# wangrui2025/GDKVM

Measured on AMD Instinct MI355X. Metric: frames/sec (GDKVM forward + argmax mask), EchoNet 112x112x32 clips, higher is better.
Workload: dtype bf16; 1 GPU; BASELINE.json configs[1]: EchoNet-Dynamic 112x112x32 bf16 inference, batch=16 per GPU; clips_per_gpu=16, frames_per_clip=32, image=112x112, heads=1, key_dim=64, rule=delta_sequential, world_size=1, ranks_seen=1

## Files before the change

### gdkvm_amd/csrc/stem_conv_pool.hip

```cpp
#include <atomic>
#include "gdkvm_common.hpp"

namespace {

constexpr int SP_TPY = 4, SP_TPX = 28;
constexpr int SP_CR = 2 * SP_TPY + 1;
constexpr int SP_CC = 64;
constexpr int SP_BR = SP_CR + 3, SP_BC = SP_CC + 3;
constexpr int SP_SLOTS = SP_BR * SP_BC * 2;
constexpr int SP_PIECES = (SP_SLOTS + 63) / 64;
constexpr int SP_BAND_BYTES = SP_PIECES * 1024;
constexpr int SP_CPIX = 144;
constexpr int SP_CONV_BYTES = SP_CR * SP_CC * SP_CPIX;

__device__ const uint4 g_stem_zero16 = {0, 0, 0, 0};

struct StemArgs {
    const bf16_t* xs; const bf16_t* w; const float* bias; bf16_t* y;
    int N, Hs, Ws, Hp, Wp, tiles_x, tiles_y;
    const bf16_t* xf; int Cf;
};

template <bool NCHW, bool POOL = true>
__global__ __launch_bounds__(512, 1) void stem_conv_pool_kernel(StemArgs a)
{
    extern __shared__ __attribute__((aligned(16))) unsigned char smem[];
    unsigned char* band2 = smem;
    unsigned char* ctile = smem + 2 * SP_BAND_BYTES;
    const int tid = threadIdx.x, lane = tid & 63, li = lane & 15, g = lane >> 4;
    const int w = __builtin_amdgcn_readfirstlane(tid >> 6), wn = w & 1, wm = w >> 1;
    const int ntiles = a.N * a.tiles_y * a.tiles_x;

    bf16x8 wf[2][8];
#pragma unroll
    for (int nt = 0; nt < 2; ++nt)
#pragma unroll
        for (int ks = 0; ks < 8; ++ks) {
            const int co = 32 * wn + 8 * (li >> 2) + 4 * nt + (li & 3);
            wf[nt][ks] = *reinterpret_cast<const bf16x8*>(a.w + (size_t)co * 256 + 32 * ks + 8 * g);
        }
    float bia[8];
    {
        const f32x4 b0 = *reinterpret_cast<const f32x4*>(a.bias + 32 * wn + 8 * g), b1 = *reinterpret_cast<const f32x4*>(a.bias + 32 * wn + 8 * g + 4);
        bia[0] = b0[0]; bia[1] = b0[1]; bia[2] = b0[2]; bia[3] = b0[3]; bia[4] = b1[0]; bia[5] = b1[1]; bia[6] = b1[2]; bia[7] = b1[3];
    }

    constexpr int PP = (SP_PIECES + 7) / 8;
    auto fetch = [&](int tile, int buf) __attribute__((always_inline)) {
        const int tx = tile % a.tiles_x, t2 = tile / a.tiles_x, ty = t2 % a.tiles_y, n = t2 / a.tiles_y;
        const int y0 = (POOL ? 2 * SP_TPY * ty - 1 : SP_CR * ty) - 2, x0 = (POOL ? 2 * SP_TPX * tx - 1 : (SP_CC - 7) * tx) - 2;
#pragma unroll
        for (int u = 0; u < PP; ++u) {
            const int j = w + 8 * u;
            if (j >= SP_PIECES) break;
            const int d = 64 * j + lane, pix = d >> 1, c = d & 1;
            const int by = pix / SP_BC, bx = pix - by * SP_BC, yy = y0 + by, xx = x0 + bx;
            const bool ok = pix < SP_BR * SP_BC && yy >= 0 && yy < a.Hs && xx >= 0 && xx < a.Ws;
            const bf16_t* src = ok ? a.xs + ((((size_t)n * a.Hs + yy) * a.Ws + xx) * 16 + c * 8) : reinterpret_cast<const bf16_t*>(&g_stem_zero16);
            __builtin_amdgcn_global_load_lds(src, reinterpret_cast<__attribute__((address_space(3))) void*>(
                reinterpret_cast<uintptr_t>(band2 + buf * SP_BAND_BYTES + 1024 * j)), 16, 0, 0);
        }
    };

    unsigned stage[PP][4];
    auto fetch_nchw = [&](int tile) __attribute__((always_inline)) {
        const int tx = tile % a.tiles_x, t2 = tile / a.tiles_x, ty = t2 % a.tiles_y, n = t2 / a.tiles_y;
        const int y0 = (POOL ? 2 * SP_TPY * ty - 1 : SP_CR * ty) - 2, x0 = (POOL ? 2 * SP_TPX * tx - 1 : (SP_CC - 7) * tx) - 2;
        const int H = 2 * a.Hs, W = 2 * a.Ws;
#pragma unroll
        for (int u = 0; u < PP; ++u) {
            const int j = w + 8 * u, d = 64 * j + lane, pix = d >> 1, half = d & 1;
            const int by = pix / SP_BC, bx = pix - by * SP_BC, yy = y0 + by, xx = x0 + bx;
            const bool ok = j < SP_PIECES && pix < SP_BR * SP_BC && yy >= 0 && yy < a.Hs && xx >= 0 && xx < a.Ws;
#pragma unroll
            for (int e = 0; e < 4; ++e) {
                const int c = 2 * half + (e >> 1);
                const bool live = ok && c < a.Cf;
                const bf16_t* src = live ? a.xf + ((((size_t)n * a.Cf + c) * H + 2 * yy + (e & 1)) * W + 2 * xx) : reinterpret_cast<const bf16_t*>(&g_stem_zero16);
                stage[u][e] = *reinterpret_cast<const unsigned*>(src);
            }
        }
    };
    auto put_nchw = [&](int buf) __attribute__((always_inline)) {
#pragma unroll
        for (int u = 0; u < PP; ++u) {
            const int j = w + 8 * u;
            if (j < SP_PIECES)
                *reinterpret_cast<uint4*>(band2 + buf * SP_BAND_BYTES + 1024 * j + 16 * lane) = make_uint4(stage[u][0], stage[u][1], stage[u][2], stage[u][3]);
        }
    };

    const unsigned xoff = (unsigned)((16 * wm + li) * 32 + g * 16);
    int tile = blockIdx.x, cur = 0;
    if (tile < ntiles) {
        if constexpr (NCHW) { fetch_nchw(tile); put_nchw(0); }
        else fetch(tile, 0);
    }
    __syncthreads();
    for (; tile < ntiles; tile += gridDim.x, cur ^= 1) {
        const bool more = tile + (int)gridDim.x < ntiles;
        if (more) {
            if constexpr (NCHW) fetch_nchw(tile + gridDim.x);
            else fetch(tile + gridDim.x, cur ^ 1);
        }
        const unsigned char* band = band2 + cur * SP_BAND_BYTES;
        const int tx = tile % a.tiles_x, t2 = tile / a.tiles_x, ty = t2 % a.tiles_y, n = t2 / a.tiles_y;
        const int cy0 = POOL ? 2 * SP_TPY * ty - 1 : SP_CR * ty, cx0 = POOL ? 2 * SP_TPX * tx - 1 : (SP_CC - 7) * tx;
        const int cx = cx0 + 16 * wm + li;
        const bool col_ok = cx >= 0 && cx < a.Ws && (POOL || 16 * wm + li < SP_CC - 7);

#pragma unroll
        for (int grp = 0; grp < 3; ++grp) {
            f32x4 acc[3][2];
#pragma unroll
            for (int r = 0; r < 3; ++r) acc[r][0] = acc[r][1] = f32x4{0.f, 0.f, 0.f, 0.f};
            bf16x8 xf[6][2];
#pragma unroll
            for (int rho = 0; rho < 6; ++rho)
#pragma unroll
                for (int half = 0; half < 2; ++half)
                    xf[rho][half] = *reinterpret_cast<const bf16x8*>(band + xoff + ((3 * grp + rho) * SP_BC) * 32 + half * 64);
#pragma unroll
            for (int ks = 0; ks < 8; ++ks) {
                const int ky = ks >> 1, half = ks & 1;
#pragma unroll
                for (int r = 0; r < 3; ++r) {
                    acc[r][0] = __builtin_amdgcn_mfma_f32_16x16x32_bf16(wf[0][ks], xf[r + ky][half], acc[r][0], 0, 0, 0);
                    acc[r][1] = __builtin_amdgcn_mfma_f32_16x16x32_bf16(wf[1][ks], xf[r + ky][half], acc[r][1], 0, 0, 0);
                }
            }
            if constexpr (!POOL) {
#pragma unroll
                for (int r = 0; r < 3; ++r) {
                    const int cy = cy0 + 3 * grp + r;
                    if (col_ok && cy < a.Hs) {
                        unsigned ow[4];
#pragma unroll
                        for (int q = 0; q < 4; ++q)
                            ow[q] = (unsigned)f32_to_bf16(acc[r][q >> 1][2 * (q & 1)]) | ((unsigned)f32_to_bf16(acc[r][q >> 1][2 * (q & 1) + 1]) << 16);
                        *reinterpret_cast<uint4*>(a.y + (((size_t)n * a.Hs + cy) * a.Ws + cx) * 64 + 32 * wn + 8 * g) = make_uint4(ow[0], ow[1], ow[2], ow[3]);
                    }
                }
                continue;
            }
#pragma unroll
            for (int r = 0; r < 3; ++r) {
                const int cr = 3 * grp + r, cy = cy0 + cr;
                const float keep = (col_ok && cy >= 0 && cy < a.Hs) ? 1.f : 0.f;
                typedef float f32x2 __attribute__((ext_vector_type(2)));
                unsigned ow[4];
#pragma unroll
                for (int q = 0; q < 4; ++q) {
                    const f32x2 t = {acc[r][q >> 1][2 * (q & 1)], acc[r][q >> 1][2 * (q & 1) + 1]};
                    const f32x2 bb = {bia[2 * q], bia[2 * q + 1]};
                    f32x2 v = __builtin_elementwise_max(t + bb, f32x2{0.f, 0.f}) * f32x2{keep, keep};
                    ow[q] = (unsigned)f32_to_bf16(v[0]) | ((unsigned)f32_to_bf16(v[1]) << 16);
                }
                *reinterpret_cast<uint4*>(ctile + (cr * SP_CC + 16 * wm + li) * SP_CPIX + (32 * wn + 8 * g) * 2) = make_uint4(ow[0], ow[1], ow[2], ow[3]);
            }
        }
        if constexpr (NCHW) { if (more) put_nchw(cur ^ 1); }
        __syncthreads();

        for (int it = tid; POOL && it < SP_TPY * SP_TPX * 8; it += 512) {
            const int cg = it & 7, pp = it >> 3, q = pp / SP_TPX, px = pp - q * SP_TPX;
            const int py_g = SP_TPY * ty + q, px_g = SP_TPX * tx + px;
            typedef unsigned short u16x2 __attribute__((ext_vector_type(2)));
            u16x2 m[4] = {u16x2{0, 0}, u16x2{0, 0}, u16x2{0, 0}, u16x2{0, 0}};
#pragma unroll
            for (int dy = 0; dy < 3; ++dy)
#pragma unroll
                for (int dx = 0; dx < 3; ++dx) {
                    const uint4 t = *reinterpret_cast<const uint4*>(ctile + ((2 * q + dy) * SP_CC + 2 * px + dx) * SP_CPIX + cg * 16);
                    m[0] = __builtin_elementwise_max(m[0], __builtin_bit_cast(u16x2, t.x));
                    m[1] = __builtin_elementwise_max(m[1], __builtin_bit_cast(u16x2, t.y));
                    m[2] = __builtin_elementwise_max(m[2], __builtin_bit_cast(u16x2, t.z));
                    m[3] = __builtin_elementwise_max(m[3], __builtin_bit_cast(u16x2, t.w));
                }
            if (py_g < a.Hp && px_g < a.Wp) {
                const uint4 o = {__builtin_bit_cast(unsigned, m[0]), __builtin_bit_cast(unsigned, m[1]), __builtin_bit_cast(unsigned, m[2]),
                                 __builtin_bit_cast(unsigned, m[3])};
                *reinterpret_cast<uint4*>(a.y + (((size_t)n * a.Hp + py_g) * a.Wp + px_g) * 64 + cg * 8) = o;
            }
        }
        if constexpr (POOL) __syncthreads();
    }
}

__global__ __launch_bounds__(256) void stem_pack_s2d_kernel(const float* w7, bf16_t* w4, int C, long long sk, long long sc, long long sr, long long ss)
{
    const int i = blockIdx.x * 256 + threadIdx.x;
    if (i >= 64 * 256) return;
    const int ch = i & 15, b = (i >> 4) & 3, a = (i >> 6) & 3, k = i >> 8;
    const int c = ch >> 2, p = (ch >> 1) & 1, q = ch & 1, u = 2 * (a - 2) + p + 3, v = 2 * (b - 2) + q + 3;
    float x = 0.f;
    if (c < C && u >= 0 && u <= 6 && v >= 0 && v <= 6) x = w7[k * sk + c * sc + u * sr + v * ss];
    w4[i] = f32_to_bf16(x);
}


constexpr int SW_TH = 4, SW_TW = 56;
constexpr int SW_BR = SW_TH + 3, SW_BC = SW_TW + 3;
constexpr int SW_BSLOTS = SW_BR * SW_BC * 2;
constexpr int SW_BPT = (SW_BSLOTS + 255) / 256;
constexpr int SW_BAND_BYTES = (SW_BSLOTS * 16 + 1023) / 1024 * 1024;
constexpr int SW_YPIX = 144;
constexpr int SW_YPIECES = (SW_TH * SW_TW * 9 + 63) / 64;
constexpr int SW_KSTEPS = SW_TH * SW_TW / 32;
static_assert(SW_TH * SW_TW % 32 == 0 && SW_TW % 4 == 0, "tiles are whole k-steps; four consecutive pixels never straddle a row");

struct StemWgradArgs { const bf16_t* xf; const bf16_t* dy; float* part; int N, Cf, Hs, Ws, tiles_x, tiles_y; };

__global__ __launch_bounds__(256, 3) void stem_wgrad_kernel(StemWgradArgs a)
{
    __shared__ __attribute__((aligned(16))) unsigned char s_band[SW_BAND_BYTES];
    __shared__ __attribute__((aligned(16))) unsigned char s_y[SW_YPIECES * 1024];
    const int tid = threadIdx.x, lane = tid & 63, li = lane & 15, g = lane >> 4;
    const int w = __builtin_amdgcn_readfirstlane(tid >> 6);
    const int q = li >> 2, p4 = (li & 3) * 4;
    const int ntiles = a.N * a.tiles_y * a.tiles_x;
    const int H = 2 * a.Hs, W = 2 * a.Ws;

    f32x4 acc[4][4];
#pragma unroll
    for (int kt = 0; kt < 4; ++kt)
#pragma unroll
        for (int b = 0; b < 4; ++b) acc[kt][b] = f32x4{0.f, 0.f, 0.f, 0.f};

    for (int tile = blockIdx.x; tile < ntiles; tile += gridDim.x) {
        const int tx = tile % a.tiles_x, t2 = tile / a.tiles_x, ty = t2 % a.tiles_y, n = t2 / a.tiles_y;
        const int cy0 = SW_TH * ty, cx0 = SW_TW * tx, y0 = cy0 - 2, x0 = cx0 - 2;
        unsigned stage[SW_BPT][4];
#pragma unroll
        for (int u = 0; u < SW_BPT; ++u) {
            const int d = 256 * u + tid, pix = d >> 1, half = d & 1;
            const int by = pix / SW_BC, bx = pix - by * SW_BC, yy = y0 + by, xx = x0 + bx;
            const bool ok = d < SW_BSLOTS && yy >= 0 && yy < a.Hs && xx >= 0 && xx < a.Ws;
#pragma unroll
            for (int e = 0; e < 4; ++e) {
                const int c = 2 * half + (e >> 1);
                const bool live = ok && c < a.Cf;
                const bf16_t* src = live ? a.xf + ((((size_t)n * a.Cf + c) * H + 2 * yy + (e & 1)) * W + 2 * xx) : reinterpret_cast<const bf16_t*>(&g_stem_zero16);
                stage[u][e] = *reinterpret_cast<const unsigned*>(src);
            }
        }
        __syncthreads();
        for (int j = w; j < SW_YPIECES; j += 4) {
            const int d = 64 * j + lane, pix = d / 9, c = d - 9 * pix;
            const int py = pix / SW_TW, px = pix - py * SW_TW, cy = cy0 + py, cx = cx0 + px;
            const bool ok = c < 8 && pix < SW_TH * SW_TW && cy < a.Hs && cx < a.Ws;
            const bf16_t* src = ok ? a.dy + ((((size_t)n * a.Hs + cy) * a.Ws + cx) * 64 + c * 8) : reinterpret_cast<const bf16_t*>(&g_stem_zero16);
            __builtin_amdgcn_global_load_lds(src, reinterpret_cast<__attribute__((address_space(3))) void*>(reinterpret_cast<uintptr_t>(s_y + 1024 * j)), 16, 0, 0);
        }
#pragma unroll
        for (int u = 0; u < SW_BPT; ++u) {
            const int d = 256 * u + tid;
            if (d < SW_BSLOTS) *reinterpret_cast<uint4*>(s_band + 16 * d) = make_uint4(stage[u][0], stage[u][1], stage[u][2], stage[u][3]);
        }
        __syncthreads();
#pragma unroll 1
        for (int s = 0; s < SW_KSTEPS; ++s) {
            unsigned ya[2], xa[2];
#pragma unroll
            for (int hf = 0; hf < 2; ++hf) {
                const int pp = 32 * s + 8 * g + 4 * hf + q, py = pp / SW_TW, px = pp - py * SW_TW;
                ya[hf] = (unsigned)(uintptr_t)(s_y + pp * SW_YPIX + p4 * 2);
                xa[hf] = (unsigned)(uintptr_t)(s_band + ((py + w) * SW_BC + px) * 32 + p4 * 2);
            }
            uint2 fa[4][2], fb[4][2];
#pragma unroll
            for (int kt = 0; kt < 4; ++kt)
#pragma unroll
                for (int hf = 0; hf < 2; ++hf) asm volatile("ds_read_b64_tr_b16 %0, %1" : "=&v"(fa[kt][hf]) : "v"(ya[hf] + 32 * kt) : "memory");
#pragma unroll
            for (int b = 0; b < 4; ++b)
#pragma unroll
                for (int hf = 0; hf < 2; ++hf) asm volatile("ds_read_b64_tr_b16 %0, %1" : "=&v"(fb[b][hf]) : "v"(xa[hf] + 32 * b) : "memory");
            asm volatile("s_waitcnt lgkmcnt(0)"
                         : "+v"(fa[0][0]), "+v"(fa[0][1]), "+v"(fa[1][0]), "+v"(fa[1][1]), "+v"(fa[2][0]), "+v"(fa[2][1]), "+v"(fa[3][0]), "+v"(fa[3][1]),
                           "+v"(fb[0][0]), "+v"(fb[0][1]), "+v"(fb[1][0]), "+v"(fb[1][1]), "+v"(fb[2][0]), "+v"(fb[2][1]), "+v"(fb[3][0]), "+v"(fb[3][1])
                         :: "memory");
#pragma unroll
            for (int b = 0; b < 4; ++b) {
                const bf16x8 bf = __builtin_bit_cast(bf16x8, make_uint4(fb[b][0].x, fb[b][0].y, fb[b][1].x, fb[b][1].y));
#pragma unroll
                for (int kt = 0; kt < 4; ++kt) {
                    const bf16x8 af = __builtin_bit_cast(bf16x8, make_uint4(fa[kt][0].x, fa[kt][0].y, fa[kt][1].x, fa[kt][1].y));
                    acc[kt][b] = __builtin_amdgcn_mfma_f32_16x16x32_bf16(af, bf, acc[kt][b], 0, 0, 0);
                }
            }
        }
    }
    float* out = a.part + (size_t)blockIdx.x * (64 * 256);
#pragma unroll
    for (int kt = 0; kt < 4; ++kt)
#pragma unroll
        for (int b = 0; b < 4; ++b)
#pragma unroll
            for (int r = 0; r < 4; ++r) out[((16 * kt + 4 * g + r) * 4 + w) * 64 + 16 * b + li] = acc[kt][b][r];
}

__global__ __launch_bounds__(512) void stem_wgrad_reduce_kernel(const float* part, float* dw, int gx, int C, long long sk, long long sc, long long sr, long long ss)
{
    __shared__ float s_sum[8][64];
    const int e = threadIdx.x & 63, sl = threadIdx.x >> 6;
    const int per = (gx + 7) / 8, b0 = sl * per, b1 = min(gx, b0 + per);
    const int i = blockIdx.x * 64 + e;
    float s8[8] = {0.f, 0.f, 0.f, 0.f, 0.f, 0.f, 0.f, 0.f};
    int b = b0;
    for (; b + 8 <= b1; b += 8)
#pragma unroll
        for (int j = 0; j < 8; ++j) s8[j] += part[(size_t)(b + j) * (64 * 256) + i];
    for (int j = 0; b < b1; ++b, ++j) s8[j] += part[(size_t)b * (64 * 256) + i];
    const float s = ((s8[0] + s8[1]) + (s8[2] + s8[3])) + ((s8[4] + s8[5]) + (s8[6] + s8[7]));
    s_sum[sl][e] = s;
    __syncthreads();
    if (sl == 0) {
        float t8 = 0.f;
#pragma unroll
        for (int j = 0; j < 8; ++j) t8 += s_sum[j][e];
        const int ch = i & 15, bb = (i >> 4) & 3, aa = (i >> 6) & 3, k = i >> 8;
        const int c = ch >> 2, p = (ch >> 1) & 1, qq = ch & 1, u = 2 * aa + p - 1, v = 2 * bb + qq - 1;
        if (c < C && u >= 0 && u <= 6 && v >= 0 && v <= 6) dw[k * sk + c * sc + u * sr + v * ss] = t8;
    }
}

}

static int stem_conv_pool_impl(const char* who, const void* xs, const void* xf, int Cf, const void* w, const float* bias, void* y,
                               int N, int Hs, int Ws, int io_dtype, void* stream, bool pool = true)
{
    if (io_dtype != GDKVM_BF16) return gdkvm_fail(GDKVM_ERR_DTYPE, "%s: only bf16 is implemented", who);
    if (N < 0 || Hs <= 0 || Ws <= 0) return gdkvm_fail(GDKVM_ERR_SHAPE, "%s: N=%d Hs=%d Ws=%d", who, N, Hs, Ws);
    if (N == 0) return GDKVM_OK;
    const void* x = xf ? xf : xs;
    if (!x || !w || (pool && !bias) || !y) return gdkvm_fail(GDKVM_ERR_ARG, "%s: null pointer", who);
    if (!gdkvm_aligned16(x) || !gdkvm_aligned16(w) || !gdkvm_aligned16(y) || (bias && !gdkvm_aligned16(bias)))
        return gdkvm_fail(GDKVM_ERR_ARG, "%s: pointers must be 16-byte aligned", who);
    if (int rc = gdkvm_check_device()) return rc;
    StemArgs a;
    a.xs = static_cast<const bf16_t*>(xs); a.w = static_cast<const bf16_t*>(w); a.bias = bias; a.y = static_cast<bf16_t*>(y);
    a.xf = static_cast<const bf16_t*>(xf); a.Cf = Cf;
    a.N = N; a.Hs = Hs; a.Ws = Ws; a.Hp = (Hs - 1) / 2 + 1; a.Wp = (Ws - 1) / 2 + 1;
    a.tiles_x = (a.Wp + SP_TPX - 1) / SP_TPX; a.tiles_y = (a.Hp + SP_TPY - 1) / SP_TPY;
    if (!pool) { a.tiles_x = (Ws + SP_CC - 8) / (SP_CC - 7); a.tiles_y = (Hs + SP_CR - 1) / SP_CR; }
    const long long ntiles = (long long)N * a.tiles_x * a.tiles_y;
    if (ntiles > 0x7fffffffLL) return gdkvm_fail(GDKVM_ERR_SHAPE, "%s: too many tiles", who);
    const size_t lds = 2 * (size_t)SP_BAND_BYTES + SP_CONV_BYTES;
    {
        static std::atomic<unsigned long long> done_mask{0};
        int dev = 0;
        if (hipGetDevice(&dev) != hipSuccess) return gdkvm_fail(GDKVM_ERR_LAUNCH, "%s: hipGetDevice", who);
        const unsigned long long bit = 1ull << (dev & 63);
        if (!(done_mask.load(std::memory_order_relaxed) & bit)) {
            hipError_t e = hipFuncSetAttribute(reinterpret_cast<const void*>(stem_conv_pool_kernel<false>), hipFuncAttributeMaxDynamicSharedMemorySize, (int)lds);
            if (e == hipSuccess) e = hipFuncSetAttribute(reinterpret_cast<const void*>(stem_conv_pool_kernel<true>), hipFuncAttributeMaxDynamicSharedMemorySize, (int)lds);
            if (e == hipSuccess) e = hipFuncSetAttribute(reinterpret_cast<const void*>(stem_conv_pool_kernel<true, false>), hipFuncAttributeMaxDynamicSharedMemorySize, (int)lds);
            if (e != hipSuccess) return gdkvm_fail(GDKVM_ERR_LAUNCH, "%s: %s", who, hipGetErrorString(e));
            done_mask.fetch_or(bit, std::memory_order_relaxed);
        }
    }
    constexpr int STEM_GRID = 256;
    const int grid = (int)(ntiles < STEM_GRID ? ntiles : STEM_GRID);
    if (!pool) hipLaunchKernelGGL((stem_conv_pool_kernel<true, false>), dim3(grid), dim3(512), lds, static_cast<hipStream_t>(stream), a);
    else if (xf) hipLaunchKernelGGL(stem_conv_pool_kernel<true>, dim3(grid), dim3(512), lds, static_cast<hipStream_t>(stream), a);
    else hipLaunchKernelGGL(stem_conv_pool_kernel<false>, dim3(grid), dim3(512), lds, static_cast<hipStream_t>(stream), a);
    GDKVM_LAUNCH_CHECK("stem_conv_pool_kernel");
    return GDKVM_OK;
}

extern "C" int gdkvm_stem_conv_pool(const void* xs, const void* w, const float* bias, void* y, int N, int Hs, int Ws,
                                    int io_dtype, void* stream)
{
    return stem_conv_pool_impl("stem_conv_pool", xs, nullptr, 0, w, bias, y, N, Hs, Ws, io_dtype, stream);
}

extern "C" int gdkvm_stem_conv_pool_nchw(const void* x, const void* w, const float* bias, void* y, int N, int C, int H, int W,
                                         int io_dtype, void* stream)
{
    if (C <= 0 || C > 4 || H <= 0 || W <= 0 || (H & 1) || (W & 1))
        return gdkvm_fail(GDKVM_ERR_SHAPE, "stem_conv_pool_nchw: C=%d H=%d W=%d (at most 4 channels, H and W even)", C, H, W);
    return stem_conv_pool_impl("stem_conv_pool_nchw", nullptr, x, C, w, bias, y, N, H / 2, W / 2, io_dtype, stream);
}

extern "C" int gdkvm_stem_conv_nchw(const void* x, const void* w4, void* y, int N, int C, int H, int W, int io_dtype, void* stream)
{
    if (C <= 0 || C > 4 || H <= 0 || W <= 0 || (H & 1) || (W & 1))
        return gdkvm_fail(GDKVM_ERR_SHAPE, "stem_conv_nchw: C=%d H=%d W=%d (at most 4 channels, H and W even)", C, H, W);
    return stem_conv_pool_impl("stem_conv_nchw", nullptr, x, C, w4, nullptr, y, N, H / 2, W / 2, io_dtype, stream, false);
}

extern "C" int gdkvm_stem_pack_s2d(const float* w7, void* w4, int C, long long sk, long long sc, long long sr, long long ss, void* stream)
{
    if (C <= 0 || C > 4) return gdkvm_fail(GDKVM_ERR_SHAPE, "stem_pack_s2d: C=%d (at most 4 input channels)", C);
    if (!w7 || !w4 || !gdkvm_aligned16(w4)) return gdkvm_fail(GDKVM_ERR_ARG, "stem_pack_s2d: null or unaligned pointer");
    if (int rc = gdkvm_check_device()) return rc;
    hipLaunchKernelGGL(stem_pack_s2d_kernel, dim3(64), dim3(256), 0, static_cast<hipStream_t>(stream), w7, static_cast<bf16_t*>(w4), C, sk, sc, sr, ss);
    GDKVM_LAUNCH_CHECK("stem_pack_s2d_kernel");
    return GDKVM_OK;
}


static int stem_wgrad_grid(int N, int Hs, int Ws, int* tiles_x, int* tiles_y)
{
    *tiles_x = (Ws + SW_TW - 1) / SW_TW; *tiles_y = (Hs + SW_TH - 1) / SW_TH;
    const long long ntiles = (long long)N * *tiles_x * *tiles_y;
    if (ntiles > 0x7fffffffLL) return -1;
    return (int)(ntiles < 768 ? ntiles : 768);
}

extern "C" size_t gdkvm_stem_wgrad_workspace_bytes(int N, int H, int W)
{
    int tx, ty;
    if (N <= 0 || H <= 0 || W <= 0) return 16;
    const int gx = stem_wgrad_grid(N, H / 2, W / 2, &tx, &ty);
    return gx <= 0 ? 16 : (size_t)gx * 64 * 256 * sizeof(float);
}

extern "C" int gdkvm_stem_wgrad_nchw(const void* x, const void* dy, float* dw, long long sk, long long sc, long long sr, long long ss,
                                     void* workspace, size_t workspace_bytes, int N, int C, int H, int W, int io_dtype, void* stream)
{
    if (io_dtype != GDKVM_BF16) return gdkvm_fail(GDKVM_ERR_DTYPE, "stem_wgrad_nchw: only bf16 operands are implemented");
    if (C <= 0 || C > 4 || H <= 0 || W <= 0 || (H & 1) || (W & 1) || N < 0)
        return gdkvm_fail(GDKVM_ERR_SHAPE, "stem_wgrad_nchw: N=%d C=%d H=%d W=%d (at most 4 channels, H and W even)", N, C, H, W);
    if (N == 0) return GDKVM_OK;
    if (!x || !dy || !dw || !workspace || !gdkvm_aligned16(x) || !gdkvm_aligned16(dy) || !gdkvm_aligned16(workspace))
        return gdkvm_fail(GDKVM_ERR_ARG, "stem_wgrad_nchw: null or unaligned pointer");
    StemWgradArgs a;
    a.xf = static_cast<const bf16_t*>(x); a.dy = static_cast<const bf16_t*>(dy); a.part = static_cast<float*>(workspace);
    a.N = N; a.Cf = C; a.Hs = H / 2; a.Ws = W / 2;
    const int gx = stem_wgrad_grid(N, a.Hs, a.Ws, &a.tiles_x, &a.tiles_y);
    if (gx <= 0) return gdkvm_fail(GDKVM_ERR_SHAPE, "stem_wgrad_nchw: too many tiles");
    const size_t need = (size_t)gx * 64 * 256 * sizeof(float);
    if (workspace_bytes < need) return gdkvm_fail(GDKVM_ERR_WORKSPACE, "stem_wgrad_nchw: workspace %zu < %zu bytes", workspace_bytes, need);
    if (int rc = gdkvm_check_device()) return rc;
    hipStream_t st = static_cast<hipStream_t>(stream);
    hipLaunchKernelGGL(stem_wgrad_kernel, dim3(gx), dim3(256), 0, st, a);
    GDKVM_LAUNCH_CHECK("stem_wgrad_kernel");
    hipLaunchKernelGGL(stem_wgrad_reduce_kernel, dim3(64 * 256 / 64), dim3(512), 0, st, static_cast<const float*>(workspace), dw, gx, C, sk, sc, sr, ss);
    GDKVM_LAUNCH_CHECK("stem_wgrad_reduce_kernel");
    return GDKVM_OK;
}
```

Baseline: 597,400 frames/s.

## Fuse stem maxpool into conv registers with row carry and DPP column max

The pooled stem kernel no longer writes the conv tile to LDS and reruns a separate pool pass. Each wave now folds conv rows straight into per-window row maxima held in registers, does the horizontal max across lanes with DPP shifts, and carries the last conv row into the next vertically adjacent tile. Tiles are handed to blocks in contiguous ranges ordered by tile row so the carry can be reused. The band is narrower (14 columns per wave), which cuts LDS use and removes the dynamic-LDS attribute setup, but lanes with odd index or index 14 and above go idle at store time, and the overlapping band columns mean some conv work is duplicated.

```diff
diff --git a/gdkvm_amd/csrc/stem_conv_pool.hip b/gdkvm_amd/csrc/stem_conv_pool.hip
--- a/gdkvm_amd/csrc/stem_conv_pool.hip
+++ b/gdkvm_amd/csrc/stem_conv_pool.hip
@@ -1,4 +1,4 @@
-#include <atomic>
+#include <type_traits>
 #include "gdkvm_common.hpp"
 
 namespace {
@@ -6,12 +6,18 @@
 constexpr int SP_TPY = 4, SP_TPX = 28;
 constexpr int SP_CR = 2 * SP_TPY + 1;
 constexpr int SP_CC = 64;
-constexpr int SP_BR = SP_CR + 3, SP_BC = SP_CC + 3;
+constexpr int SP_BR = SP_CR + 3;
+
+constexpr int SP_CS = 14;
+constexpr int SPP_BC = 3 * SP_CS + 16 + 3;
+constexpr int SPP_PIECES = (SP_BR * SPP_BC * 2 + 63) / 64;
+constexpr int SPP_BAND_BYTES = SPP_PIECES * 1024;
+static_assert(SP_TPX == 4 * (SP_CS / 2) && SP_CS % 2 == 0, "each wave pools SP_CS / 2 whole windows");
+
+constexpr int SP_BC = SP_CC + 3;
 constexpr int SP_SLOTS = SP_BR * SP_BC * 2;
 constexpr int SP_PIECES = (SP_SLOTS + 63) / 64;
 constexpr int SP_BAND_BYTES = SP_PIECES * 1024;
-constexpr int SP_CPIX = 144;
-constexpr int SP_CONV_BYTES = SP_CR * SP_CC * SP_CPIX;
 
 __device__ const uint4 g_stem_zero16 = {0, 0, 0, 0};
 
@@ -21,15 +27,16 @@
     const bf16_t* xf; int Cf;
 };
 
-template <bool NCHW, bool POOL = true>
+template <bool NCHW>
 __global__ __launch_bounds__(512, 1) void stem_conv_pool_kernel(StemArgs a)
 {
     extern __shared__ __attribute__((aligned(16))) unsigned char smem[];
     unsigned char* band2 = smem;
-    unsigned char* ctile = smem + 2 * SP_BAND_BYTES;
     const int tid = threadIdx.x, lane = tid & 63, li = lane & 15, g = lane >> 4;
     const int w = __builtin_amdgcn_readfirstlane(tid >> 6), wn = w & 1, wm = w >> 1;
     const int ntiles = a.N * a.tiles_y * a.tiles_x;
+    const int per = (ntiles + (int)gridDim.x - 1) / (int)gridDim.x;
+    const int t0 = (int)blockIdx.x * per, t1 = min(ntiles, t0 + per);
 
     bf16x8 wf[2][8];
 #pragma unroll
@@ -45,27 +52,180 @@
         bia[0] = b0[0]; bia[1] = b0[1]; bia[2] = b0[2]; bia[3] = b0[3]; bia[4] = b1[0]; bia[5] = b1[1]; bia[6] = b1[2]; bia[7] = b1[3];
     }
 
-    constexpr int PP = (SP_PIECES + 7) / 8;
-    auto fetch = [&](int tile, int buf) __attribute__((always_inline)) {
-        const int tx = tile % a.tiles_x, t2 = tile / a.tiles_x, ty = t2 % a.tiles_y, n = t2 / a.tiles_y;
-        const int y0 = (POOL ? 2 * SP_TPY * ty - 1 : SP_CR * ty) - 2, x0 = (POOL ? 2 * SP_TPX * tx - 1 : (SP_CC - 7) * tx) - 2;
+    auto where = [&](int t, int& n, int& ty, int& tx) __attribute__((always_inline)) {
+        ty = t % a.tiles_y; const int t2 = t / a.tiles_y; tx = t2 % a.tiles_x; n = t2 / a.tiles_x;
+    };
+    constexpr int PP = (SPP_PIECES + 7) / 8;
+    auto fetch = [&](int t, int buf) __attribute__((always_inline)) {
+        int n, ty, tx; where(t, n, ty, tx);
+        const int y0 = 2 * SP_TPY * ty - 3, x0 = 2 * SP_TPX * tx - 3;
 #pragma unroll
         for (int u = 0; u < PP; ++u) {
             const int j = w + 8 * u;
-            if (j >= SP_PIECES) break;
+            if (j >= SPP_PIECES) break;
             const int d = 64 * j + lane, pix = d >> 1, c = d & 1;
-            const int by = pix / SP_BC, bx = pix - by * SP_BC, yy = y0 + by, xx = x0 + bx;
-            const bool ok = pix < SP_BR * SP_BC && yy >= 0 && yy < a.Hs && xx >= 0 && xx < a.Ws;
+            const int by = pix / SPP_BC, bx = pix - by * SPP_BC, yy = y0 + by, xx = x0 + bx;
+            const bool ok = pix < SP_BR * SPP_BC && yy >= 0 && yy < a.Hs && xx >= 0 && xx < a.Ws;
             const bf16_t* src = ok ? a.xs + ((((size_t)n * a.Hs + yy) * a.Ws + xx) * 16 + c * 8) : reinterpret_cast<const bf16_t*>(&g_stem_zero16);
             __builtin_amdgcn_global_load_lds(src, reinterpret_cast<__attribute__((address_space(3))) void*>(
-                reinterpret_cast<uintptr_t>(band2 + buf * SP_BAND_BYTES + 1024 * j)), 16, 0, 0);
+                reinterpret_cast<uintptr_t>(band2 + buf * SPP_BAND_BYTES + 1024 * j)), 16, 0, 0);
         }
     };
 
+    unsigned stage[PP][4];
+    auto fetch_nchw = [&](int t) __attribute__((always_inline)) {
+        int n, ty, tx; where(t, n, ty, tx);
+        const int y0 = 2 * SP_TPY * ty - 3, x0 = 2 * SP_TPX * tx - 3;
+        const int H = 2 * a.Hs, W = 2 * a.Ws;
+#pragma unroll
+        for (int u = 0; u < PP; ++u) {
+            const int j = w + 8 * u, d = 64 * j + lane, pix = d >> 1, half = d & 1;
+            const int by = pix / SPP_BC, bx = pix - by * SPP_BC, yy = y0 + by, xx = x0 + bx;
+            const bool ok = j < SPP_PIECES && pix < SP_BR * SPP_BC && yy >= 0 && yy < a.Hs && xx >= 0 && xx < a.Ws;
+#pragma unroll
+            for (int e = 0; e < 4; ++e) {
+                const int c = 2 * half + (e >> 1);
+                const bool live = ok && c < a.Cf;
+                const bf16_t* src = live ? a.xf + ((((size_t)n * a.Cf + c) * H + 2 * yy + (e & 1)) * W + 2 * xx) : reinterpret_cast<const bf16_t*>(&g_stem_zero16);
+                stage[u][e] = *(const __attribute__((address_space(1))) unsigned*)src;
+            }
+        }
+    };
+    auto put_nchw = [&](int buf) __attribute__((always_inline)) {
+#pragma unroll
+        for (int u = 0; u < PP; ++u) {
+            const int j = w + 8 * u;
+            if (j < SPP_PIECES)
+                *reinterpret_cast<uint4*>(band2 + buf * SPP_BAND_BYTES + 1024 * j + 16 * lane) = make_uint4(stage[u][0], stage[u][1], stage[u][2], stage[u][3]);
+        }
+    };
+
+    typedef unsigned short u16x2 __attribute__((ext_vector_type(2)));
+    const unsigned xoff = (unsigned)((SP_CS * wm + li) * 32 + g * 16);
+    if (t0 < t1) {
+        if constexpr (NCHW) { fetch_nchw(t0); put_nchw(0); }
+        else fetch(t0, 0);
+    }
+    __syncthreads();
+    u16x2 carry[4];
+    int cur = 0;
+    for (int t = t0; t < t1; ++t, cur ^= 1) {
+        const bool more = t + 1 < t1;
+        if (more) {
+            if constexpr (NCHW) fetch_nchw(t + 1);
+            else fetch(t + 1, cur ^ 1);
+        }
+        const unsigned char* band = band2 + cur * SPP_BAND_BYTES;
+        int n, ty, tx; where(t, n, ty, tx);
+        const bool carried = t > t0 && ty > 0;
+        const int cy0 = 2 * SP_TPY * ty - 1;
+        const int cx = 2 * SP_TPX * tx - 1 + SP_CS * wm + li;
+        const bool col_ok = cx >= 0 && cx < a.Ws;
+
+        u16x2 pm[SP_TPY][4];
+#pragma unroll
+        for (int q = 0; q < SP_TPY; ++q)
+#pragma unroll
+            for (int i = 0; i < 4; ++i) pm[q][i] = u16x2{0, 0};
+        auto fold = [&](int cr, const u16x2 (&v)[4]) __attribute__((always_inline)) {
+#pragma unroll
+            for (int q = 0; q < SP_TPY; ++q)
+                if (2 * q <= cr && cr <= 2 * q + 2)
+#pragma unroll
+                    for (int i = 0; i < 4; ++i) pm[q][i] = __builtin_elementwise_max(pm[q][i], v[i]);
+            if (cr == SP_CR - 1)
+#pragma unroll
+                for (int i = 0; i < 4; ++i) carry[i] = v[i];
+        };
+        auto rows = [&](auto r0c, auto nrc) __attribute__((always_inline)) {
+            constexpr int R0 = decltype(r0c)::value, NR = decltype(nrc)::value;
+            f32x4 acc[NR][2];
+#pragma unroll
+            for (int r = 0; r < NR; ++r) acc[r][0] = acc[r][1] = f32x4{0.f, 0.f, 0.f, 0.f};
+#pragma unroll
+            for (int rho = 0; rho < NR + 3; ++rho) {
+                const bf16x8 x0 = *reinterpret_cast<const bf16x8*>(band + xoff + ((R0 + rho) * SPP_BC) * 32);
+                const bf16x8 x1 = *reinterpret_cast<const bf16x8*>(band + xoff + ((R0 + rho) * SPP_BC) * 32 + 64);
+#pragma unroll
+                for (int r = 0; r < NR; ++r) {
+                    const int ky = rho - r;
+                    if (ky < 0 || ky > 3) continue;
+                    acc[r][0] = __builtin_amdgcn_mfma_f32_16x16x32_bf16(wf[0][2 * ky], x0, acc[r][0], 0, 0, 0);
+                    acc[r][1] = __builtin_amdgcn_mfma_f32_16x16x32_bf16(wf[1][2 * ky], x0, acc[r][1], 0, 0, 0);
+                    acc[r][0] = __builtin_amdgcn_mfma_f32_16x16x32_bf16(wf[0][2 * ky + 1], x1, acc[r][0], 0, 0, 0);
+                    acc[r][1] = __builtin_amdgcn_mfma_f32_16x16x32_bf16(wf[1][2 * ky + 1], x1, acc[r][1], 0, 0, 0);
+                }
+            }
+#pragma unroll
+            for (int r = 0; r < NR; ++r) {
+                const int cr = R0 + r, cy = cy0 + cr;
+                const float keep = (col_ok && cy >= 0 && cy < a.Hs) ? 1.f : 0.f;
+                u16x2 v[4];
+#pragma unroll
+                for (int q = 0; q < 4; ++q) {
+                    const float e0 = __builtin_fmaxf(acc[r][q >> 1][2 * (q & 1)] + bia[2 * q], 0.f) * keep;
+                    const float e1 = __builtin_fmaxf(acc[r][q >> 1][2 * (q & 1) + 1] + bia[2 * q + 1], 0.f) * keep;
+                    v[q] = u16x2{f32_to_bf16(e0), f32_to_bf16(e1)};
+                }
+                fold(cr, v);
+            }
+        };
+        auto emit = [&](int q) __attribute__((always_inline)) {
+            unsigned o[4];
+#pragma unroll
+            for (int i = 0; i < 4; ++i) {
+                const int m = __builtin_bit_cast(int, pm[q][i]);
+                const int r1 = __builtin_amdgcn_update_dpp(0, m, 0x101, 0xf, 0xf, true);
+                const int r2 = __builtin_amdgcn_update_dpp(0, m, 0x102, 0xf, 0xf, true);
+                o[i] = __builtin_bit_cast(unsigned, __builtin_elementwise_max(__builtin_elementwise_max(pm[q][i], __builtin_bit_cast(u16x2, r1)),
+                                                                              __builtin_bit_cast(u16x2, r2)));
+            }
+            const int py = SP_TPY * ty + q, px = SP_TPX * tx + (SP_CS / 2) * wm + (li >> 1);
+            if (!(li & 1) && li < SP_CS && py < a.Hp && px < a.Wp)
+                *reinterpret_cast<uint4*>(a.y + (((size_t)n * a.Hp + py) * a.Wp + px) * 64 + 32 * wn + 8 * g) = make_uint4(o[0], o[1], o[2], o[3]);
+        };
+
+        if (carried) fold(0, carry);
+        else rows(std::integral_constant<int, 0>{}, std::integral_constant<int, 1>{});
+        rows(std::integral_constant<int, 1>{}, std::integral_constant<int, 3>{});
+        emit(0);
+        rows(std::integral_constant<int, 4>{}, std::integral_constant<int, 3>{});
+        emit(1);
+        emit(2);
+        rows(std::integral_constant<int, 7>{}, std::integral_constant<int, 2>{});
+        emit(3);
+
+        if constexpr (NCHW) {
+            if (more) put_nchw(cur ^ 1);
+            asm volatile("s_waitcnt lgkmcnt(0)\n\ts_barrier" ::: "memory");
+        } else {
+            __syncthreads();
+        }
+    }
+}
+
+__global__ __launch_bounds__(512, 1) void stem_conv_kernel(StemArgs a)
+{
+    extern __shared__ __attribute__((aligned(16))) unsigned char smem[];
+    unsigned char* band2 = smem;
+    const int tid = threadIdx.x, lane = tid & 63, li = lane & 15, g = lane >> 4;
+    const int w = __builtin_amdgcn_readfirstlane(tid >> 6), wn = w & 1, wm = w >> 1;
+    const int ntiles = a.N * a.tiles_y * a.tiles_x;
+
+    bf16x8 wf[2][8];
+#pragma unroll
+    for (int nt = 0; nt < 2; ++nt)
+#pragma unroll
+        for (int ks = 0; ks < 8; ++ks) {
+            const int co = 32 * wn + 8 * (li >> 2) + 4 * nt + (li & 3);
+            wf[nt][ks] = *reinterpret_cast<const bf16x8*>(a.w + (size_t)co * 256 + 32 * ks + 8 * g);
+        }
+
+    constexpr int PP = (SP_PIECES + 7) / 8;
     unsigned stage[PP][4];
     auto fetch_nchw = [&](int tile) __attribute__((always_inline)) {
         const int tx = tile % a.tiles_x, t2 = tile / a.tiles_x, ty = t2 % a.tiles_y, n = t2 / a.tiles_y;
-        const int y0 = (POOL ? 2 * SP_TPY * ty - 1 : SP_CR * ty) - 2, x0 = (POOL ? 2 * SP_TPX * tx - 1 : (SP_CC - 7) * tx) - 2;
+        const int y0 = SP_CR * ty - 2, x0 = (SP_CC - 7) * tx - 2;
         const int H = 2 * a.Hs, W = 2 * a.Ws;
 #pragma unroll
         for (int u = 0; u < PP; ++u) {
@@ -92,22 +252,16 @@
 
     const unsigned xoff = (unsigned)((16 * wm + li) * 32 + g * 16);
     int tile = blockIdx.x, cur = 0;
-    if (tile < ntiles) {
-        if constexpr (NCHW) { fetch_nchw(tile); put_nchw(0); }
-        else fetch(tile, 0);
-    }
+    if (tile < ntiles) { fetch_nchw(tile); put_nchw(0); }
     __syncthreads();
     for (; tile < ntiles; tile += gridDim.x, cur ^= 1) {
         const bool more = tile + (int)gridDim.x < ntiles;
-        if (more) {
-            if constexpr (NCHW) fetch_nchw(tile + gridDim.x);
-            else fetch(tile + gridDim.x, cur ^ 1);
-        }
+        if (more) fetch_nchw(tile + gridDim.x);
         const unsigned char* band = band2 + cur * SP_BAND_BYTES;
         const int tx = tile % a.tiles_x, t2 = tile / a.tiles_x, ty = t2 % a.tiles_y, n = t2 / a.tiles_y;
-        const int cy0 = POOL ? 2 * SP_TPY * ty - 1 : SP_CR * ty, cx0 = POOL ? 2 * SP_TPX * tx - 1 : (SP_CC - 7) * tx;
+        const int cy0 = SP_CR * ty, cx0 = (SP_CC - 7) * tx;
         const int cx = cx0 + 16 * wm + li;
-        const bool col_ok = cx >= 0 && cx < a.Ws && (POOL || 16 * wm + li < SP_CC - 7);
+        const bool col_ok = cx >= 0 && cx < a.Ws && 16 * wm + li < SP_CC - 7;
 
 #pragma unroll
         for (int grp = 0; grp < 3; ++grp) {
@@ -129,61 +283,20 @@
                     acc[r][1] = __builtin_amdgcn_mfma_f32_16x16x32_bf16(wf[1][ks], xf[r + ky][half], acc[r][1], 0, 0, 0);
                 }
             }
-            if constexpr (!POOL) {
-#pragma unroll
-                for (int r = 0; r < 3; ++r) {
-                    const int cy = cy0 + 3 * grp + r;
-                    if (col_ok && cy < a.Hs) {
-                        unsigned ow[4];
-#pragma unroll
-                        for (int q = 0; q < 4; ++q)
-                            ow[q] = (unsigned)f32_to_bf16(acc[r][q >> 1][2 * (q & 1)]) | ((unsigned)f32_to_bf16(acc[r][q >> 1][2 * (q & 1) + 1]) << 16);
-                        *reinterpret_cast<uint4*>(a.y + (((size_t)n * a.Hs + cy) * a.Ws + cx) * 64 + 32 * wn + 8 * g) = make_uint4(ow[0], ow[1], ow[2], ow[3]);
-                    }
+#pragma unroll
+            for (int r = 0; r < 3; ++r) {
+                const int cy = cy0 + 3 * grp + r;
+                if (col_ok && cy < a.Hs) {
+                    unsigned ow[4];
+#pragma unroll
+                    for (int q = 0; q < 4; ++q)
+                        ow[q] = (unsigned)f32_to_bf16(acc[r][q >> 1][2 * (q & 1)]) | ((unsigned)f32_to_bf16(acc[r][q >> 1][2 * (q & 1) + 1]) << 16);
+                    *reinterpret_cast<uint4*>(a.y + (((size_t)n * a.Hs + cy) * a.Ws + cx) * 64 + 32 * wn + 8 * g) = make_uint4(ow[0], ow[1], ow[2], ow[3]);
                 }
-                continue;
-            }
-#pragma unroll
-            for (int r = 0; r < 3; ++r) {
-                const int cr = 3 * grp + r, cy = cy0 + cr;
-                const float keep = (col_ok && cy >= 0 && cy < a.Hs) ? 1.f : 0.f;
-                typedef float f32x2 __attribute__((ext_vector_type(2)));
-                unsigned ow[4];
-#pragma unroll
-                for (int q = 0; q < 4; ++q) {
-                    const f32x2 t = {acc[r][q >> 1][2 * (q & 1)], acc[r][q >> 1][2 * (q & 1) + 1]};
-                    const f32x2 bb = {bia[2 * q], bia[2 * q + 1]};
-                    f32x2 v = __builtin_elementwise_max(t + bb, f32x2{0.f, 0.f}) * f32x2{keep, keep};
-                    ow[q] = (unsigned)f32_to_bf16(v[0]) | ((unsigned)f32_to_bf16(v[1]) << 16);
-                }
-                *reinterpret_cast<uint4*>(ctile + (cr * SP_CC + 16 * wm + li) * SP_CPIX + (32 * wn + 8 * g) * 2) = make_uint4(ow[0], ow[1], ow[2], ow[3]);
-            }
-        }
-        if constexpr (NCHW) { if (more) put_nchw(cur ^ 1); }
+            }
+        }
+        if (more) put_nchw(cur ^ 1);
         __syncthreads();
-
-        for (int it = tid; POOL && it < SP_TPY * SP_TPX * 8; it += 512) {
-            const int cg = it & 7, pp = it >> 3, q = pp / SP_TPX, px = pp - q * SP_TPX;
-            const int py_g = SP_TPY * ty + q, px_g = SP_TPX * tx + px;
-            typedef unsigned short u16x2 __attribute__((ext_vector_type(2)));
-            u16x2 m[4] = {u16x2{0, 0}, u16x2{0, 0}, u16x2{0, 0}, u16x2{0, 0}};
-#pragma unroll
-            for (int dy = 0; dy < 3; ++dy)
-#pragma unroll
-                for (int dx = 0; dx < 3; ++dx) {
-                    const uint4 t = *reinterpret_cast<const uint4*>(ctile + ((2 * q + dy) * SP_CC + 2 * px + dx) * SP_CPIX + cg * 16);
-                    m[0] = __builtin_elementwise_max(m[0], __builtin_bit_cast(u16x2, t.x));
-                    m[1] = __builtin_elementwise_max(m[1], __builtin_bit_cast(u16x2, t.y));
-                    m[2] = __builtin_elementwise_max(m[2], __builtin_bit_cast(u16x2, t.z));
-                    m[3] = __builtin_elementwise_max(m[3], __builtin_bit_cast(u16x2, t.w));
-                }
-            if (py_g < a.Hp && px_g < a.Wp) {
-                const uint4 o = {__builtin_bit_cast(unsigned, m[0]), __builtin_bit_cast(unsigned, m[1]), __builtin_bit_cast(unsigned, m[2]),
-                                 __builtin_bit_cast(unsigned, m[3])};
-                *reinterpret_cast<uint4*>(a.y + (((size_t)n * a.Hp + py_g) * a.Wp + px_g) * 64 + cg * 8) = o;
-            }
-        }
-        if constexpr (POOL) __syncthreads();
     }
 }
 
@@ -346,25 +459,18 @@
     if (!pool) { a.tiles_x = (Ws + SP_CC - 8) / (SP_CC - 7); a.tiles_y = (Hs + SP_CR - 1) / SP_CR; }
     const long long ntiles = (long long)N * a.tiles_x * a.tiles_y;
     if (ntiles > 0x7fffffffLL) return gdkvm_fail(GDKVM_ERR_SHAPE, "%s: too many tiles", who);
-    const size_t lds = 2 * (size_t)SP_BAND_BYTES + SP_CONV_BYTES;
-    {
-        static std::atomic<unsigned long long> done_mask{0};
-        int dev = 0;
-        if (hipGetDevice(&dev) != hipSuccess) return gdkvm_fail(GDKVM_ERR_LAUNCH, "%s: hipGetDevice", who);
-        const unsigned long long bit = 1ull << (dev & 63);
-        if (!(done_mask.load(std::memory_order_relaxed) & bit)) {
-            hipError_t e = hipFuncSetAttribute(reinterpret_cast<const void*>(stem_conv_pool_kernel<false>), hipFuncAttributeMaxDynamicSharedMemorySize, (int)lds);
-            if (e == hipSuccess) e = hipFuncSetAttribute(reinterpret_cast<const void*>(stem_conv_pool_kernel<true>), hipFuncAttributeMaxDynamicSharedMemorySize, (int)lds);
-            if (e == hipSuccess) e = hipFuncSetAttribute(reinterpret_cast<const void*>(stem_conv_pool_kernel<true, false>), hipFuncAttributeMaxDynamicSharedMemorySize, (int)lds);
-            if (e != hipSuccess) return gdkvm_fail(GDKVM_ERR_LAUNCH, "%s: %s", who, hipGetErrorString(e));
-            done_mask.fetch_or(bit, std::memory_order_relaxed);
-        }
-    }
     constexpr int STEM_GRID = 256;
-    const int grid = (int)(ntiles < STEM_GRID ? ntiles : STEM_GRID);
-    if (!pool) hipLaunchKernelGGL((stem_conv_pool_kernel<true, false>), dim3(grid), dim3(512), lds, static_cast<hipStream_t>(stream), a);
-    else if (xf) hipLaunchKernelGGL(stem_conv_pool_kernel<true>, dim3(grid), dim3(512), lds, static_cast<hipStream_t>(stream), a);
-    else hipLaunchKernelGGL(stem_conv_pool_kernel<false>, dim3(grid), dim3(512), lds, static_cast<hipStream_t>(stream), a);
+    hipStream_t st = static_cast<hipStream_t>(stream);
+    if (!pool) {
+        const int grid = (int)(ntiles < STEM_GRID ? ntiles : STEM_GRID);
+        hipLaunchKernelGGL(stem_conv_kernel, dim3(grid), dim3(512), 2 * SP_BAND_BYTES, st, a);
+        GDKVM_LAUNCH_CHECK("stem_conv_kernel");
+        return GDKVM_OK;
+    }
+    const long long per = (ntiles + STEM_GRID - 1) / STEM_GRID;
+    const int grid = (int)((ntiles + per - 1) / per);
+    if (xf) hipLaunchKernelGGL(stem_conv_pool_kernel<true>, dim3(grid), dim3(512), 2 * SPP_BAND_BYTES, st, a);
+    else hipLaunchKernelGGL(stem_conv_pool_kernel<false>, dim3(grid), dim3(512), 2 * SPP_BAND_BYTES, st, a);
     GDKVM_LAUNCH_CHECK("stem_conv_pool_kernel");
     return GDKVM_OK;
 }
```

Measured after the change: 606,800 frames/s (median of 6 runs). 1.02x the previous value.
